# dusk-network/plonk_gadgets

Measured on AMD Instinct MI355X. Metric: gadget constraints/sec (range_check 256-bit), higher is better.
Workload: dtype u64x4 (BLS12-381 scalar, Montgomery limbs)

## Files before the change

### plonk_gadgets_amd/csrc/capi_composer.inc

```

struct RaggedBuffers {
    Scratch row_off, var_off, num_bits;
    uint64_t *rows() const { return row_off.as<uint64_t>(); }
    uint64_t *vars() const { return var_off.as<uint64_t>(); }
    uint32_t *bits() const { return num_bits.as<uint32_t>(); }
};

struct pg_composer {
    pg_engine *e = nullptr;
    hipStream_t stream = nullptr;
    uint64_t n = 0, nvars = 0, zero_var = 0;
    ColumnStore cols;
    Scratch d_stage;
    uint64_t *stage_words() const { return d_stage.as<uint64_t>(); }
    std::vector<uint64_t> pi_gate;
    std::vector<pg_scalar> pi_val;
    std::vector<pg::FourthWire> fourth;
    std::vector<pg::RangeSeg> range_segs;
    std::vector<pg::PermSeg> segs;
    Scratch perm_small, perm_big, val_ws;
    Scratch perm_pieces;
    std::vector<RaggedBuffers> ragged;
    Pinned h_total;
    uint64_t *totals() const { return h_total.as<uint64_t>(); }
// ... 1404 lines not shown
    if (np) {
        PG_TRY(B.take(d_gate, np * 8));
        PG_TRY(B.take(d_val, np * 32));
        PG_HIP_TRY(hipMemcpyAsync(*d_gate, c->pi_gate.data(), np * 8, hipMemcpyHostToDevice, c->stream));
        PG_HIP_TRY(hipMemcpyAsync(*d_val, c->pi_val.data(), np * 32, hipMemcpyHostToDevice, c->stream));
    }
    if (nf) {
        PG_TRY(B.take(d_fw, nf * sizeof(pg::FourthWire)));
        PG_HIP_TRY(hipMemcpyAsync(*d_fw, c->fourth.data(), nf * sizeof(pg::FourthWire), hipMemcpyHostToDevice, c->stream));
    }
    return PG_OK;
}

pg_status pg_composer_check(pg_composer *c, int64_t *first_bad) {
    if (!c || !first_bad) return fail(PG_ERR_INVALID_ARGUMENT, "NULL argument");
    PG_TRY(flush(c));
    PG_HIP_TRY(hipSetDevice(c->e->device));
    CallBuffers B(c->stream);
    uint64_t *d_gate; uint4 *d_val; pg::FourthWire *d_fw;
    PG_TRY(upload_sparse(c, B, &d_gate, &d_val, &d_fw));
    unsigned long long *d_bad = nullptr, h_bad = ~0ull;
    PG_TRY(B.take(&d_bad, 8));
    PG_HIP_TRY(hipMemcpyAsync(d_bad, &h_bad, 8, hipMemcpyHostToDevice, c->stream));
    const uint64_t want = (c->n + pg::kThreads - 1) / pg::kThreads;
    const uint32_t grid = (uint32_t)(want < (uint64_t)c->e->num_cus * 8 ? (want ? want : 1) : (uint64_t)c->e->num_cus * 8);
    hipLaunchKernelGGL(pg::check_kernel, dim3(grid), dim3(pg::kThreads), 0, c->stream, c->cols.view(), c->n, (uint64_t)0, c->nvars,
                       c->zero_var, d_gate, d_val, (uint32_t)c->pi_gate.size(), d_fw, (uint32_t)c->fourth.size(), d_bad);
    for (const pg::RangeSeg &s : c->range_segs) {
        const uint64_t rw = (s.items * s.g + pg::kThreads - 1) / pg::kThreads, most = (uint64_t)c->e->num_cus * 8;
        hipLaunchKernelGGL(pg::range_check_rows_kernel, dim3((uint32_t)(rw < most ? rw : most)), dim3(pg::kThreads), 0, c->stream, c->cols.view(), s,
                           c->nvars, d_bad);
    }
    PG_HIP_TRY(hipGetLastError());
    PG_HIP_TRY(hipMemcpyAsync(&h_bad, d_bad, 8, hipMemcpyDeviceToHost, c->stream));
    PG_HIP_TRY(hipStreamSynchronize(c->stream));
    *first_bad = h_bad == ~0ull ? -1 : (int64_t)h_bad;
    return PG_OK;
}

pg_status pg_composer_dense_pi(pg_composer *c, pg_scalar *d_out) {
    if (!c) return fail(PG_ERR_INVALID_ARGUMENT, "composer is NULL");
    PG_TRY(flush(c));
    PG_TRY(check_scalars(d_out, "d_out"));
    PG_HIP_TRY(hipSetDevice(c->e->device));
    PG_HIP_TRY(hipMemsetAsync(d_out, 0, c->n * 32, c->stream));
    CallBuffers B(c->stream);
    uint64_t *d_gate; uint4 *d_val; pg::FourthWire *d_fw;
    PG_TRY(upload_sparse(c, B, &d_gate, &d_val, &d_fw));
    const uint32_t np = (uint32_t)c->pi_gate.size();
    if (np) {
        hipLaunchKernelGGL(pg::scatter_pi_kernel, dim3((np + 255) / 256), dim3(256), 0, c->stream,
                           reinterpret_cast<uint4 *>(d_out), d_gate, d_val, np);
        PG_HIP_TRY(hipGetLastError());
    }
    PG_HIP_TRY(hipStreamSynchronize(c->stream));
    return PG_OK;
}

pg_status pg_composer_materialize(pg_composer *c, const pg_full_columns *out) {
    if (!c || !out) return fail(PG_ERR_INVALID_ARGUMENT, "NULL argument");
    PG_TRY(flush(c));
    PG_HIP_TRY(hipSetDevice(c->e->device));
    const uint32_t grid = (uint32_t)c->e->num_cus * 32;
    pg::MaterializeOut M{};
    pg_scalar *const consts[7] = {out->q_4, out->q_arith, out->q_range, out->q_logic, out->q_fixed_group_add,
                                  out->q_variable_group_add, out->w_4_value};
    for (int k = 0; k < 7; k++) {
        if (!consts[k]) continue;
        PG_TRY(check_scalars(consts[k], "constant column"));
        M.konst[k] = reinterpret_cast<uint4 *>(consts[k]);
    }
    pg_scalar *const vals[3] = {out->w_l_value, out->w_r_value, out->w_o_value};
    for (int i = 0; i < 3; i++) {
        if (!vals[i]) continue;
        PG_TRY(check_scalars(vals[i], "wire value column"));
        M.val[i] = reinterpret_cast<uint4 *>(vals[i]);
    }
    if (out->w_4) {
        PG_TRY(check_u64s(out->w_4, "w_4"));
        M.w_4 = out->w_4;
    }
    const auto generic = [&](uint64_t lo, uint64_t hi) {
        if (hi <= lo) return;
        const uint64_t want = (2 * (hi - lo) + 16383) / 16384;
        hipLaunchKernelGGL(pg::materialize_kernel, dim3((uint32_t)(want < grid ? want : grid)), dim3(pg::kThreads), 0, c->stream, c->cols.view(), M,
                           lo, hi, c->zero_var);
    };
    uint64_t at = 0;
#ifndef PG_MAT_GRID_PER_CU
#define PG_MAT_GRID_PER_CU 64
#endif
    using MatKernel = void (*)(const pg::ComposerCols, const pg::MaterializeOut, const pg::PermSeg, uint32_t, uint64_t);
    static const MatKernel self_ragged[2] = {pg::materialize_items_kernel<pg::MAT_SELF, pg::WIRES_MAX_BOUND, true>,
                                             pg::materialize_items_kernel<pg::MAT_SELF, pg::WIRES_MIX, true>};
    static const MatKernel read_wires = pg::materialize_items_kernel<pg::MAT_READ_WIRES, pg::WIRES_UNKNOWN>;
    static const MatKernel self[pg::WIRES_MIX + 1] = {
        nullptr,
        pg::materialize_items_kernel<pg::MAT_SELF, pg::WIRES_RANGE_CHECK>,
        pg::materialize_items_kernel<pg::MAT_SELF, pg::WIRES_MAX_BOUND>,
        pg::materialize_items_kernel<pg::MAT_SELF, pg::WIRES_RANGE_CHECK_ALLOCATED>,
        pg::materialize_items_kernel<pg::MAT_SELF, pg::WIRES_MAX_BOUND_ALLOCATED>,
        pg::materialize_items_kernel<pg::MAT_SELF, pg::WIRES_DECOMPOSITION>,
        pg::materialize_items_kernel<pg::MAT_SELF, pg::WIRES_MIX>,
    };
    for (const pg::PermSeg &s : c->segs) {
        const uint64_t group = pg::mat_group(s);
        const pg::MatRoute r = pg::mat_route(s, group);
        if (!r.windowed) continue;
        generic(at, s.gate_base);
        const uint64_t n_groups = (s.items + group - 1) / group, most = (uint64_t)c->e->num_cus * PG_MAT_GRID_PER_CU;
        const MatKernel kernel = r.mode != pg::MAT_SELF ? read_wires : r.ragged ? self_ragged[r.kind == pg::WIRES_MIX] : self[r.kind];
        hipLaunchKernelGGL(kernel, dim3((uint32_t)(n_groups < most ? n_groups : most)), dim3(pg::kMatThreads), 0, c->stream, c->cols.view(), M, s,
                           (uint32_t)group, c->zero_var);
        at = s.gate_end;
    }
    generic(at, c->n);
    CallBuffers B(c->stream);
    uint64_t *d_gate; uint4 *d_val; pg::FourthWire *d_fw;
    PG_TRY(upload_sparse(c, B, &d_gate, &d_val, &d_fw));
    if (d_fw)
        hipLaunchKernelGGL(pg::patch_fourth_kernel, dim3(1), dim3(64), 0, c->stream, reinterpret_cast<uint4 *>(out->q_4), out->w_4,
                           reinterpret_cast<uint4 *>(out->w_4_value), c->cols.view().vars, d_fw, (uint32_t)c->fourth.size());
    if (out->q_range)
        for (const pg::RangeSeg &s : c->range_segs) {
            const uint64_t rw = (2 * s.items * s.g + pg::kThreads - 1) / pg::kThreads;
            hipLaunchKernelGGL(pg::range_patch_kernel, dim3((uint32_t)(rw < grid ? rw : grid)), dim3(pg::kThreads), 0, c->stream,
                               reinterpret_cast<uint4 *>(out->q_range), s);
        }
    PG_HIP_TRY(hipGetLastError());
    PG_HIP_TRY(hipStreamSynchronize(c->stream));
    return PG_OK;
}

static pg_status perm_reserve(pg_composer *c, Scratch &buf, size_t bytes) {
    if (bytes <= buf.size()) return PG_OK;
    PG_HIP_TRY(hipStreamSynchronize(c->stream));
    return buf.reserve(bytes);
}

pg_status pg_composer_permutation_reserve(pg_composer *c, uint64_t sparse_positions) {
    if (!c) return fail(PG_ERR_INVALID_ARGUMENT, "composer is NULL");
    c->sparse_cap_first = sparse_positions;
    if (sparse_positions) c->perm_last_sparse = 0;
    return PG_OK;
}

static pg_status perm_kernel_attributes(pg_engine *e) {
    if (e->perm_attributes_set) return PG_OK;
    const void *const ladder_lds[4] = {
        reinterpret_cast<const void *>(pg::perm_ladder_kernel<false>), reinterpret_cast<const void *>(pg::perm_template_kernel<true>),
        reinterpret_cast<const void *>(pg::perm_template_kernel<false>), reinterpret_cast<const void *>(pg::perm_ladder_kernel<true>)};
    if (pg::kPermLadderLds)
        for (const void *k : ladder_lds) PG_HIP_TRY(hipFuncSetAttribute(k, hipFuncAttributeMaxDynamicSharedMemorySize, (int)pg::kPermLadderLds));
    PG_HIP_TRY(hipFuncSetAttribute(reinterpret_cast<const void *>(pg::perm_identity_kernel), hipFuncAttributeMaxDynamicSharedMemorySize,
                                   (int)pg::kPermIdentityLds));
    e->perm_attributes_set = true;
    return PG_OK;
}

pg_status pg_composer_permutation(pg_composer *c, uint64_t padded_n, uint64_t *d_sigma) {
    if (!c) return fail(PG_ERR_INVALID_ARGUMENT, "composer is NULL");
    PG_TRY(flush(c));
    PG_TRY(check_u64s(d_sigma, "d_sigma"));
    if (padded_n < c->n) return fail(PG_ERR_INVALID_ARGUMENT, "padded_n is smaller than the circuit");
    PG_HIP_TRY(hipSetDevice(c->e->device));
    PG_TRY(perm_kernel_attributes(c->e));
    const uint32_t grid = (uint32_t)c->e->num_cus * 32;
    uint32_t pos_bits = 2, var_bits = 1;
    while ((1ull << pos_bits) < 4 * c->n) pos_bits++;
    while ((1ull << var_bits) < c->nvars + 1) var_bits++;
    if (pos_bits + var_bits > 64) return fail(PG_ERR_INVALID_ARGUMENT, "circuit too large for 64-bit (Variable, position) keys");
    std::vector<pg::PermSeg> segs;
    std::vector<pg::PermRoute> routes;
    std::vector<std::pair<uint64_t, uint64_t>> gaps;
    uint64_t at = 0, gap_rows = 0;
    for (pg::PermSeg s : c->segs) {
        const pg::PermRoute route = pg::perm_route(s);
        if (!(s.group = pg::perm_group(s, route))) continue;
        if (s.gate_base > at) gaps.emplace_back(at, s.gate_base);
        segs.push_back(s);
        routes.push_back(route);
        at = s.gate_end;
    }
    if (c->n > at) gaps.emplace_back(at, c->n);
    for (const auto &g : gaps) gap_rows += g.second - g.first;
    const size_t seg_bytes = round256(segs.size() * sizeof(pg::PermSeg));
    const size_t fw_bytes = round256(c->fourth.size() * sizeof(pg::FourthWire));
    PG_TRY(perm_reserve(c, c->perm_small, seg_bytes + fw_bytes + 256));
    char *small = c->perm_small.as<char>();
    pg::PermCtx X;
    X.C = c->cols.view(); X.n = c->n; X.padded_n = padded_n; X.zero_var = c->zero_var;
    X.segs = reinterpret_cast<const pg::PermSeg *>(small); X.n_segs = (uint32_t)segs.size();
    X.fw = reinterpret_cast<const pg::FourthWire *>(small + seg_bytes); X.n_fw = (uint32_t)c->fourth.size();
    X.fw_lo = 0; X.fw_span = 0; X.pos_bits = pos_bits;
    X.hole_key = pos_bits + var_bits >= 64 ? ~0ull : (1ull << (pos_bits + var_bits)) - 1;
    if (!c->fourth.empty()) {
        uint64_t lo = ~0ull, hi = 0;
        for (const pg::FourthWire &f : c->fourth) { lo = f.gate < lo ? f.gate : lo; hi = f.gate > hi ? f.gate : hi; }
        X.fw_lo = lo; X.fw_span = hi - lo;
    }
    uint64_t reserved = 0, total_pieces = 0;
    for (size_t i = 0; i < segs.size(); i++) {
        if (pg::perm_reserves_slots(routes[i])) {
            segs[i].sparse_base = reserved;
            reserved += segs[i].items * pg::perm_slots_per_item(segs[i], routes[i]);
        }
        if (pg::perm_needs_piece_items(routes[i])) total_pieces += pg::perm_pieces(segs[i]);
    }
    if (total_pieces) {
        PG_TRY(perm_reserve(c, c->perm_pieces, total_pieces * sizeof(uint32_t)));
        uint32_t *at_piece = c->perm_pieces.as<uint32_t>();
        for (size_t i = 0; i < segs.size(); i++) {
            if (!pg::perm_needs_piece_items(routes[i])) continue;
            pg::PermSeg &s = segs[i];
            s.piece_item = at_piece;
            at_piece += pg::perm_pieces(s);
            const uint64_t want = (s.items + pg::kThreads - 1) / pg::kThreads;
            hipLaunchKernelGGL(pg::perm_piece_items_kernel, dim3((uint32_t)(want < grid ? want : grid)), dim3(pg::kThreads), 0, c->stream, s,
                               pg::kPermLadderRows, at_piece - pg::perm_pieces(s));
        }
        PG_HIP_TRY(hipGetLastError());
    }
    unsigned long long *d_count = reinterpret_cast<unsigned long long *>(small + seg_bytes + fw_bytes);
    if (!segs.empty())
        PG_HIP_TRY(hipMemcpyAsync(small, segs.data(), segs.size() * sizeof(pg::PermSeg), hipMemcpyHostToDevice, c->stream));
    if (!c->fourth.empty())
        PG_HIP_TRY(hipMemcpyAsync(small + seg_bytes, c->fourth.data(), c->fourth.size() * sizeof(pg::FourthWire),
                                  hipMemcpyHostToDevice, c->stream));
    uint64_t cap = c->sparse_cap_first ? c->sparse_cap_first : 4 * gap_rows + c->sparse_hint + (1ull << 16), nS = 0;
    if (cap < c->perm_last_sparse) cap = c->perm_last_sparse;
    uint64_t *k0 = nullptr, *k1 = nullptr, holes = 0;
    size_t tmp_bytes = 0;
    for (int attempt = 0;; attempt++) {
        uint64_t *nul = nullptr;
        PG_HIP_TRY(rocprim::radix_sort_keys(nullptr, tmp_bytes, nul, nul, (size_t)cap, 0u, pos_bits + var_bits, c->stream));
        const size_t kb = round256(cap * 8);
        PG_TRY(perm_reserve(c, c->perm_big, 2 * kb + tmp_bytes + 256));
        k0 = c->perm_big.as<uint64_t>();
        k1 = reinterpret_cast<uint64_t *>(c->perm_big.as<char>() + kb);
        const pg::PermSparse Q{k0, d_count, cap};
        hipLaunchKernelGGL(pg::perm_count_init_kernel, dim3(1), dim3(1), 0, c->stream, d_count, reserved);
        for (size_t i = 0; i < segs.size(); i++) {
            const pg::PermSeg &s = segs[i];
            const uint64_t most = (uint64_t)c->e->num_cus * 64, pieces = pg::perm_pieces(s);
            const uint32_t lds = pg::perm_lds_bytes(s, routes[i]);
            if (routes[i] != pg::PERM_ITEMS && routes[i] != pg::PERM_LADDER && pieces > 0x7fffffffull)
                return fail(PG_ERR_INVALID_ARGUMENT, "segment too large for one launch");
            switch (routes[i]) {
            case pg::PERM_LADDER: {
                const uint64_t lmost = pg::kPermLadderRows <= 2048 ? 0x7fffffffull : most;
                hipLaunchKernelGGL(pg::perm_ladder_kernel<false>, dim3((uint32_t)(pieces < lmost ? pieces : lmost)), dim3(pg::kThreads), lds,
                                   c->stream, X, s, Q, d_sigma);
                break;
            }
            case pg::PERM_LADDER_RAGGED:
                hipLaunchKernelGGL(pg::perm_ladder_kernel<true>, dim3((uint32_t)pieces), dim3(pg::kThreads), lds, c->stream, X, s, Q, d_sigma);
                break;
            case pg::PERM_TEMPLATE:
                hipLaunchKernelGGL(pg::perm_template_kernel<false>, dim3((uint32_t)pieces), dim3(pg::kThreads), lds, c->stream, X, s,
                                   pg::template_rows(s.wire_kind), Q, d_sigma);
                break;
            case pg::PERM_TEMPLATE_RAGGED:
                hipLaunchKernelGGL(pg::perm_template_kernel<true>, dim3((uint32_t)pieces), dim3(pg::kThreads), lds, c->stream, X, s,
                                   pg::template_rows(s.wire_kind), Q, d_sigma);
                break;
            case pg::PERM_ITEMS: {
                const uint64_t groups = (s.items + s.group - 1) / s.group;
                hipLaunchKernelGGL(pg::perm_item_kernel, dim3((uint32_t)(groups < most ? groups : most)), dim3(pg::kThreads), lds, c->stream, X, s,
                                   groups, Q, d_sigma);
                break;
            }
            }
        }
        for (const auto &g : gaps) {
            const uint64_t nblk = (g.second - g.first + pg::kPermChunk - 1) / pg::kPermChunk;
            hipLaunchKernelGGL(pg::perm_gap_kernel, dim3((uint32_t)nblk), dim3(pg::kThreads), 0, c->stream, X, g.first, g.second, Q,
                               d_sigma);
        }
        PG_HIP_TRY(hipMemcpyAsync(c->totals(), d_count, 16, hipMemcpyDeviceToHost, c->stream));
        PG_HIP_TRY(hipStreamSynchronize(c->stream));
        nS = c->totals()[0];
        holes = c->totals()[1];
        c->perm_last_sparse = nS;
        if (nS <= cap) break;
        if (attempt) return fail(PG_ERR_HIP, "sparse position list grew between two passes");
        cap = nS;
    }
    if (nS) {
        PG_HIP_TRY(rocprim::radix_sort_keys(c->perm_big.as<char>() + 2 * round256(cap * 8), tmp_bytes, k0, k1,
                                            (size_t)nS, 0u, pos_bits + var_bits, c->stream));
        nS -= holes;
    }
    if (nS) {
        const uint64_t want = (nS + pg::kThreads - 1) / pg::kThreads;
        hipLaunchKernelGGL(pg::perm_sparse_link_kernel, dim3((uint32_t)(want < grid ? want : grid)), dim3(pg::kThreads), 0, c->stream,
                           X, k1, nS, d_sigma);
        if (!segs.empty()) {
            const uint64_t wantw = (nS + 255) / 256;
            hipLaunchKernelGGL(pg::perm_splice_kernel, dim3((uint32_t)(wantw < grid ? wantw : grid)), dim3(pg::kThreads), 0, c->stream,
                               X, k1, nS, d_sigma);
        }
    }
    if (padded_n > c->n) {
        const uint64_t per_run = ((padded_n - c->n) / 2 + 1 + pg::kPermIdentityUnits - 1) / pg::kPermIdentityUnits;
        if (4 * per_run > 0x7fffffffull) return fail(PG_ERR_INVALID_ARGUMENT, "padding too large for one launch");
        hipLaunchKernelGGL(pg::perm_identity_kernel, dim3((uint32_t)(4 * per_run)), dim3(pg::kThreads), pg::kPermIdentityLds, c->stream,
                           d_sigma, c->n, padded_n);
    }
    PG_HIP_TRY(hipGetLastError());
    return PG_OK;
}

pg_status pg_check_rows(pg_engine *e, const pg_columns *cols, uint64_t n_gates, uint64_t var_base, uint64_t n_vars,
                        pg_variable zero_var, int64_t *first_bad, void *stream) {
    if (!e || !first_bad) return fail(PG_ERR_INVALID_ARGUMENT, "NULL argument");
    *first_bad = -1;
    if (n_gates == 0) return PG_OK;
    PG_TRY(check_columns(cols));
    PG_HIP_TRY(hipSetDevice(e->device));
    hipStream_t st = static_cast<hipStream_t>(stream);
    pg::ComposerCols C;
    C.q[0] = reinterpret_cast<uint4 *>(cols->q_m); C.q[1] = reinterpret_cast<uint4 *>(cols->q_l);
    C.q[2] = reinterpret_cast<uint4 *>(cols->q_r); C.q[3] = reinterpret_cast<uint4 *>(cols->q_o);
    C.q[4] = reinterpret_cast<uint4 *>(cols->q_c);
    C.w[0] = cols->w_l; C.w[1] = cols->w_r; C.w[2] = cols->w_o;
    C.vars = reinterpret_cast<uint4 *>(cols->var_values);
    unsigned long long *d_bad = nullptr, h_bad = ~0ull;
    CallBuffers B(st);
    PG_TRY(B.take(&d_bad, 8));
    PG_HIP_TRY(hipMemcpyAsync(d_bad, &h_bad, 8, hipMemcpyHostToDevice, st));
    hipLaunchKernelGGL(pg::check_kernel, dim3((uint32_t)e->num_cus * 16), dim3(pg::kThreads), 0, st, C, n_gates, var_base, n_vars,
                       zero_var, (const uint64_t *)nullptr, (const uint4 *)nullptr, 0u, (const pg::FourthWire *)nullptr, 0u, d_bad);
    hipError_t le = hipGetLastError();
    if (le == hipSuccess) le = hipMemcpyAsync(&h_bad, d_bad, 8, hipMemcpyDeviceToHost, st);
    if (le == hipSuccess) le = hipStreamSynchronize(st);
    if (le != hipSuccess) return fail(PG_ERR_HIP, std::string("pg_check_rows: ") + hipGetErrorString(le));
    *first_bad = h_bad == ~0ull ? -1 : (int64_t)h_bad;
    return PG_OK;
}

}
```

### plonk_gadgets_amd/csrc/experiment.hpp

```cpp
#pragma once

#if !defined(PG_EXPERIMENT) &&                                                                                                  \
    (defined(PG_NT_STORES) || defined(PG_FULL_BARRIERS) || defined(PG_EMIT_WAVES_PER_SIMD) || defined(PG_XCD_REMAP) ||          \
     defined(PG_UNALIGNED_SWEEPS) || defined(PG_ROWS_WAVES_PER_SIMD) || defined(PG_ROWS_SETPRIO) || defined(PG_INVERT_FERMAT) || \
     defined(PG_INV_GRP) || defined(PG_RC_W) || defined(PG_MB_W) || defined(PG_MIX_VARS_VGPRS) || defined(PG_MIX_STAMPS) ||     \
     defined(PG_QUEUE_MAX) || defined(PG_PERM_LDS_PAD) || defined(PG_GRID_BLOCKS_PER_CU) || defined(PG_PLAN_TWO_LAUNCHES) ||    \
     defined(PG_INV_LANES_PER_CU) || defined(PG_INV_MAX_PER_LANE) || defined(PG_SIDE_STREAM_NORMAL_PRIORITY) || defined(PG_VAR_SWEEP_SINGLE) || \
     defined(PG_TILE_SPREAD) || defined(PG_MIX_EARLY_TILES) || defined(PG_MAT_THREADS) || defined(PG_MAT_UNROLL) || defined(PG_MAT_LOADS) || defined(PG_PERM_LADDER_ROWS) || defined(PG_PERM_LADDER_LDS) || defined(PG_MAT_GRID_PER_CU) || defined(PG_EMIT_GRID_BLOCKS_PER_CU) || \
     defined(PG_MSM_SMALL_WINDOW))
#error "a PG_... build option is defined without -DPG_EXPERIMENT: the shipped library is built with none of them (csrc/experiment.hpp)"
#endif
```

### plonk_gadgets_amd/csrc/footprint.hpp

```cpp
#pragma once

#include <cstdint>

#if defined(__HIPCC__)
#define PG_FOOTPRINT_HD __host__ __device__
#else
#define PG_FOOTPRINT_HD
#endif

namespace pg {

struct PermSeg {
    uint64_t gate_base, gate_end, var_base, var_end;
    uint32_t L, V;
    uint64_t items;
    const uint64_t *row_off, *var_off;
    uint32_t group;
    uint32_t wire_kind, wire_n;
    uint64_t sparse_base;
    uint32_t tail;
    const uint32_t *piece_item;
};
enum : uint32_t { WIRES_UNKNOWN = 0, WIRES_RANGE_CHECK = 1, WIRES_MAX_BOUND = 2, WIRES_RANGE_CHECK_ALLOCATED = 3, WIRES_MAX_BOUND_ALLOCATED = 4,
                  WIRES_DECOMPOSITION = 5,
                  WIRES_MIX = 6,
                  WIRES_SELECT_ZERO = 7, WIRES_SELECT_ONE = 8, WIRES_MAYBE_EQUAL = 9, WIRES_IS_NON_ZERO = 10, WIRES_GATE_OUT = 11,
                  WIRES_GATE_ROWS = 12, WIRES_KINDS = 13 };

PG_FOOTPRINT_HD inline uint32_t ladder_foreign_per_item(uint32_t kind) {
    return kind == WIRES_RANGE_CHECK_ALLOCATED ? 4u : kind == WIRES_MAX_BOUND_ALLOCATED ? 2u : kind == WIRES_DECOMPOSITION ? 1u : 0u;
}
PG_FOOTPRINT_HD inline uint32_t template_foreign_per_item(uint32_t kind) {
    return kind == WIRES_SELECT_ZERO || kind == WIRES_MAYBE_EQUAL || kind == WIRES_IS_NON_ZERO || kind == WIRES_GATE_OUT ? 2u
           : kind == WIRES_SELECT_ONE || kind == WIRES_GATE_ROWS ? 3u : 0u;
}
PG_FOOTPRINT_HD inline bool is_template_kind(uint32_t kind) { return kind >= WIRES_MIX && kind < WIRES_KINDS; }

struct KindShape {
    uint16_t rows, rows_per_bit, vars, vars_per_bit;
    uint8_t allocated_twin;
};
constexpr KindShape kKindShapes[WIRES_KINDS] = {
    {0, 0, 0, 0, 0},
    {11, 4, 524, 2, WIRES_RANGE_CHECK_ALLOCATED},
    {5, 2, 262, 1, WIRES_MAX_BOUND_ALLOCATED},
    {11, 4, 523, 2, 0},
    {5, 2, 261, 1, 0},
    {4, 2, 260, 1, 0},
    {10, 0, 15, 0, 0},
    {1, 0, 1, 0, 0},
    {4, 0, 4, 0, 0},
    {3, 0, 3, 0, 0},
    {3, 0, 3, 0, 0},
    {1, 0, 1, 0, 0},
    {1, 0, 0, 0, 0},
};
constexpr uint32_t kind_rows(uint32_t kind, uint64_t n = 0) { return kKindShapes[kind].rows + kKindShapes[kind].rows_per_bit * (uint32_t)n; }
constexpr uint32_t kind_vars(uint32_t kind, uint64_t n = 0) { return kKindShapes[kind].vars + kKindShapes[kind].vars_per_bit * (uint32_t)n; }
constexpr uint32_t ladder_kind(uint32_t fused_kind, bool fused) { return fused ? fused_kind : kKindShapes[fused_kind].allocated_twin; }
inline uint32_t kind_foreign(uint32_t kind) { return is_template_kind(kind) ? template_foreign_per_item(kind) : ladder_foreign_per_item(kind); }
inline uint32_t kind_sparse_hint(uint32_t kind) { return kind == WIRES_DECOMPOSITION ? 2u : kind_foreign(kind); }

inline PermSeg footprint(uint64_t gate0, uint64_t var0, uint64_t items, uint32_t wire_kind, uint32_t wire_n = 0, uint32_t tail = 0) {
    const uint32_t L = kind_rows(wire_kind, wire_n) + tail, V = kind_vars(wire_kind, wire_n);
    return PermSeg{gate0, gate0 + items * L, var0, var0 + items * V, L, V, items, nullptr, nullptr, 1, wire_kind, wire_n, 0, tail, nullptr};
}

constexpr uint32_t kFootprintMinRows = 4096;

constexpr uint32_t kPermLocalLdsLimit = 64 * 1024 - 256;
constexpr uint32_t kPermNone = 0xFFFF, kPermDone = 0xFFFE;
PG_FOOTPRINT_HD inline uint32_t perm_local_lds_bytes(uint32_t L, uint32_t V) {
    return 4 * V + 2 * (V + 2) + 2 * (3 * L + 3 * L + L) + L + 16;
}
#ifndef PG_PERM_LADDER_ROWS
#define PG_PERM_LADDER_ROWS 512
#endif
#ifndef PG_PERM_LADDER_LDS
#define PG_PERM_LADDER_LDS 39936
#endif
#ifndef PG_PERM_LDS_PAD
#define PG_PERM_LDS_PAD 0
#endif
constexpr uint32_t kPermLadderRows = PG_PERM_LADDER_ROWS;
constexpr uint32_t kPermLadderLds = PG_PERM_LADDER_LDS;

enum PermRoute : uint32_t {
    PERM_ITEMS = 0,
    PERM_LADDER,
    PERM_LADDER_RAGGED,
    PERM_TEMPLATE,
    PERM_TEMPLATE_RAGGED,
};
inline PermRoute perm_route(const PermSeg &s) {
    if (s.wire_kind != WIRES_UNKNOWN && !s.row_off && s.wire_n >= 2) return PERM_LADDER;
    if (is_template_kind(s.wire_kind) && s.tail == 0) return s.row_off ? PERM_TEMPLATE_RAGGED : PERM_TEMPLATE;
    if (s.row_off && s.wire_kind == WIRES_MAX_BOUND && s.tail == 0) return PERM_LADDER_RAGGED;
    return PERM_ITEMS;
}
inline bool perm_fits(const PermSeg &s, uint64_t k) {
    return 4 * k * s.L < kPermDone && k * s.V < kPermNone && perm_local_lds_bytes((uint32_t)(k * s.L), (uint32_t)(k * s.V)) <= kPermLocalLdsLimit;
}
inline uint32_t perm_group(const PermSeg &s, PermRoute route) {
    if (!perm_fits(s, 1)) return 0;
    if (route == PERM_LADDER ? !is_template_kind(s.wire_kind) || s.tail == 0 : route != PERM_ITEMS) return 1;
    uint64_t k = 1024 / s.L;
    k = k < 1 ? 1 : (k > s.items ? s.items : k);
    while (k > 1 && !perm_fits(s, k)) k--;
    return (uint32_t)k;
}
inline bool perm_reserves_slots(PermRoute route) { return route == PERM_LADDER || route == PERM_TEMPLATE || route == PERM_TEMPLATE_RAGGED; }
inline uint32_t perm_slots_per_item(const PermSeg &s, PermRoute route) {
    return route == PERM_LADDER ? ladder_foreign_per_item(s.wire_kind) : perm_reserves_slots(route) ? template_foreign_per_item(s.wire_kind) : 0u;
}
inline bool perm_needs_piece_items(PermRoute route) { return route == PERM_LADDER_RAGGED || route == PERM_TEMPLATE_RAGGED; }
inline uint64_t perm_pieces(const PermSeg &s) { return (s.gate_end - (s.gate_base & ~1ull) + kPermLadderRows - 1) / kPermLadderRows; }
inline uint32_t perm_lds_bytes(const PermSeg &s, PermRoute route) {
    switch (route) {
    case PERM_LADDER: return ladder_foreign_per_item(s.wire_kind) ? 0u : kPermLadderLds;
    case PERM_LADDER_RAGGED: return kPermLadderLds;
    case PERM_TEMPLATE:
    case PERM_TEMPLATE_RAGGED: return template_foreign_per_item(s.wire_kind) ? 0u : kPermLadderLds - 8192;
    default: return perm_local_lds_bytes(s.group * s.L, s.group * s.V) + PG_PERM_LDS_PAD;
    }
}

constexpr uint32_t kMatWindowVars = 1040;
enum : int {
    MAT_READ_WIRES = 0,
    MAT_SELF = 2,
};
constexpr uint32_t kMatWitItems = 4;
constexpr uint32_t kMatMixRaggedItems = 127;

inline uint64_t mat_group(const PermSeg &s) {
    const uint64_t group = kMatWindowVars / (s.V ? s.V : 1);
    return group < 1 ? 1 : (group > s.items ? s.items : group);
}
struct MatRoute {
    bool windowed;
    int mode;
    uint32_t kind;
    bool ragged;
};
inline MatRoute mat_route(const PermSeg &s, uint64_t group) {
    if (s.V > kMatWindowVars || s.V == 0 || s.gate_end - s.gate_base < kFootprintMinRows) return MatRoute{false, MAT_READ_WIRES, WIRES_UNKNOWN, false};
    if (s.row_off) {
        if (s.wire_kind == WIRES_MAX_BOUND && group <= kMatWitItems) return MatRoute{true, MAT_SELF, WIRES_MAX_BOUND, true};
        if (s.wire_kind == WIRES_MIX && group < kMatMixRaggedItems) return MatRoute{true, MAT_SELF, WIRES_MIX, true};
        return MatRoute{true, MAT_READ_WIRES, WIRES_UNKNOWN, false};
    }
    if (s.wire_kind != WIRES_UNKNOWN && s.wire_kind <= WIRES_MIX && (ladder_foreign_per_item(s.wire_kind) == 0 || group <= kMatWitItems))
        return MatRoute{true, MAT_SELF, s.wire_kind, false};
    return MatRoute{true, MAT_READ_WIRES, WIRES_UNKNOWN, false};
}

}
```

### plonk_gadgets_amd/csrc/permutation.hpp

```cpp
#pragma once

#include <cstring>

#include <rocprim/rocprim.hpp>

#include "composer.hpp"
#include "footprint.hpp"
#include "range_gadgets.hpp"

namespace pg {

constexpr uint32_t kZeroWire = 0xfffffffeu;
__device__ __forceinline__ void seg_wire_offsets(uint32_t kind, uint32_t n, uint32_t j, uint32_t off[3], uint32_t tail = 0) {
    const uint32_t x0 = kind == WIRES_RANGE_CHECK || kind == WIRES_MAX_BOUND ? 1u : 0u;
    if (tail && kind >= WIRES_RANGE_CHECK && kind <= WIRES_MAX_BOUND_ALLOCATED) {
        const bool rc = kind == WIRES_RANGE_CHECK || kind == WIRES_RANGE_CHECK_ALLOCATED;
        const uint32_t own = rc ? 4 * n + 11 : 2 * n + 5, res = x0 + (rc ? 2 * n + 522 : n + 260);
        if (j >= own) {
            off[0] = off[1] = off[2] = res;
            return;
        }
    }
    if (kind == WIRES_MIX) {
        constexpr uint64_t lo = 0xF50ull | 0x777ull << 12 | 0x760ull << 24 | 0x888ull << 36 | 0x921ull << 48;
// ... 332 lines not shown
    }
    const uint32_t open = ladder_block_row(j, n, j2, w2);
    if (j == 0) {
        if (kind == WIRES_MAX_BOUND_ALLOCATED) return 3;
        j2[0] = 0; w2[0] = 1; j2[1] = 0; w2[1] = 0;
    } else if (open == 2) { j2[1] = 0; w2[1] = 2; }
    else if (open == 1) { j2[0] = tail ? L : 2 * n + 3; w2[0] = tail ? 0 : 2; }
    return 0;
}

__device__ __forceinline__ uint32_t ladder_foreign_wires(uint32_t kind, uint32_t n, uint32_t j) {
    if (kind == WIRES_RANGE_CHECK_ALLOCATED) return j == 0 || j == 2 * n + 5 ? 3u : 0u;
    if (kind == WIRES_MAX_BOUND_ALLOCATED) return j == 0 ? 3u : 0u;
    if (kind == WIRES_DECOMPOSITION) return j == 2 * n + 1 ? 2u : 0u;
    return 0u;
}

__device__ __forceinline__ uint32_t ladder_foreign_rank(uint32_t kind, uint32_t j, uint32_t w) {
    if (kind == WIRES_DECOMPOSITION) return 0u;
    return (j ? 2u : 0u) + w;
}

constexpr uint32_t kPermRaggedWindow = 64;
__global__ __launch_bounds__(kThreads) void perm_piece_items_kernel(const PermSeg S, uint32_t rows_per_piece, uint32_t *piece_item) {
    const uint64_t d = S.gate_base & 1;
    for (uint64_t i = (uint64_t)blockIdx.x * kThreads + threadIdx.x; i < S.items; i += (uint64_t)gridDim.x * kThreads) {
        const uint64_t r0 = S.row_off[i], r1 = S.row_off[i + 1];
        if (i == 0) piece_item[0] = 0;
        for (uint64_t p = (r0 + d + rows_per_piece - 1) / rows_per_piece; p * rows_per_piece < r1 + d; p++)
            if (p) piece_item[p] = (uint32_t)i;
    }
}

template <bool RAGGED>
__global__ __launch_bounds__(kThreads) void perm_ladder_kernel(const PermCtx X, const PermSeg S, const PermSparse Q, uint64_t *sigma) {
    extern __shared__ uint4 perm_ladder_pad[];
    __shared__ uint32_t s_off[RAGGED ? kPermRaggedWindow : 1];
    static_assert(!RAGGED || kPermLadderRows / 9 + 3 <= kPermRaggedWindow, "a piece's items fit the window of prefix sums");
    const uint32_t lane = threadIdx.x & 63, kind = S.wire_kind;
    uint32_t n = S.wire_n;
    if (X.padded_n == 1) perm_ladder_pad[threadIdx.x] = make_uint4(0, 0, 0, 0);
    const uint64_t first = S.gate_base & ~1ull, total = S.gate_end - first;
    const bool wide = (reinterpret_cast<uintptr_t>(sigma) & 15) == 0 && !(X.padded_n & 1);
    const uint32_t recip = (uint32_t)(((1ull << 32) + S.L - 1) / S.L);
    const bool pow2 = (X.padded_n & (X.padded_n - 1)) == 0;
    const uint32_t sh = 63u - (uint32_t)__clzll((long long)X.padded_n);
    auto enc = [&](uint64_t gate, uint32_t wire) { return pow2 ? ((uint64_t)wire << sh) + gate : perm_encode(gate, wire, X.padded_n); };
    auto zero_wires = [&](uint64_t g, uint32_t j) {
        uint32_t z = 0;
        for (uint32_t m = ladder_foreign_wires(kind, n, j); m; m &= m - 1) {
            const uint32_t w = (uint32_t)__ffs((int)m) - 1;
            if (X.C.w[w][g] == X.zero_var) z |= 1u << w;
        }
        return z;
    };
    for (uint64_t base = (uint64_t)blockIdx.x * kPermLadderRows; base < total; base += (uint64_t)gridDim.x * kPermLadderRows) {
        const uint64_t g_first = first + base, rel = g_first < S.gate_base ? 0 : g_first - S.gate_base;
        uint64_t item0, rows0 = 0;
        if constexpr (RAGGED) {
            item0 = S.piece_item[base / kPermLadderRows];
            rows0 = S.row_off[item0];
            __syncthreads();
            if (threadIdx.x < kPermRaggedWindow) {
                const uint64_t i = item0 + threadIdx.x < S.items ? item0 + threadIdx.x : S.items;
                s_off[threadIdx.x] = (uint32_t)(S.row_off[i] - rows0);
            }
            __syncthreads();
        } else {
            item0 = rel / S.L;
            rows0 = item0 * S.L;
        }
        const uint32_t j0 = (uint32_t)(rel - rows0), skip = (uint32_t)(g_first < S.gate_base ? S.gate_base - g_first : 0);
        for (uint32_t t = 2 * threadIdx.x; t < kPermLadderRows; t += 2 * kThreads) {
            uint64_t out[4][2], fitem[2] = {0, 0};
            uint32_t foreign[2] = {0, 0}, fslots[2] = {0, 0}, fj[2] = {0, 0};
            bool live[2];
#pragma unroll
            for (uint32_t h = 0; h < 2; h++) {
                const uint64_t g = g_first + t + h;
                live[h] = g >= S.gate_base && g < S.gate_end;
                const uint32_t tt = t + h - skip;
                uint32_t q, j;
                uint64_t g_item;
#pragma unroll
                for (uint32_t w = 0; w < 4; w++) out[w][h] = 0;
                if constexpr (RAGGED) {
                    if (!live[h]) continue;
                    const uint32_t x = j0 + tt;
                    uint32_t lo = 0;
#pragma unroll
                    for (uint32_t step = kPermRaggedWindow / 2; step; step >>= 1)
                        if (s_off[lo + step] <= x) lo += step;
                    q = lo;
                    j = x - s_off[lo];
                    n = (s_off[lo + 1] - s_off[lo] - 5) >> 1;
                    g_item = S.gate_base + rows0 + s_off[lo];
                } else {
                    q = __umulhi(j0 + tt, recip);
                    j = (j0 + tt) - q * S.L;
                    g_item = S.gate_base + (item0 + q) * S.L;
                }
                if (!live[h]) continue;
                uint32_t j2[3], w2[3];
                const uint32_t fw = ladder_row(kind, n, j, j2, w2, S.tail), zw = fw ? zero_wires(g, j) : 0u;
                foreign[h] = fw & ~zw;
                fslots[h] = fw;
                fitem[h] = item0 + q;
                fj[h] = j;
#pragma unroll
                for (uint32_t w = 0; w < 3; w++) {
                    if (fw >> w & 1) {
                        const uint32_t later = (zw | 8u) & ~((2u << w) - 1);
                        out[w][h] = enc(g, (uint32_t)__ffs((int)later) - 1);
                    } else {
                        out[w][h] = enc(g_item + j2[w], w2[w]);
                    }
                }
                if (g + 1 < S.gate_end) {
                    const uint32_t jn = j + 1 == S.L ? 0 : j + 1;
                    const uint32_t zn = ladder_foreign_wires(kind, n, jn) ? zero_wires(g + 1, jn) : 0u;
                    out[3][h] = enc(g + 1, (uint32_t)__ffs((int)(zn | 8u)) - 1);
                } else {
                    out[3][h] = perm_next_zero_from(X, S.gate_end);
                }
            }
            const uint64_t g = g_first + t;
#pragma unroll
            for (uint32_t w = 0; w < 4; w++) {
                const bool skip0 = !live[0] || (foreign[0] >> w & 1), skip1 = !live[1] || (foreign[1] >> w & 1);
                uint64_t *dst = sigma + enc(g, w);
                if (wide && !skip0 && !skip1)
                    store16(reinterpret_cast<uint4 *>(dst), make_uint4((uint32_t)out[w][0], (uint32_t)(out[w][0] >> 32), (uint32_t)out[w][1],
                                                                      (uint32_t)(out[w][1] >> 32)));
                else {
                    if (!skip0) dst[0] = out[w][0];
                    if (!skip1) dst[1] = out[w][1];
                }
            }
            if (fslots[0] | fslots[1]) {
                const uint32_t F = ladder_foreign_per_item(kind);
#pragma unroll
                for (uint32_t h = 0; h < 2; h++)
                    for (uint32_t m = fslots[h]; m; m &= m - 1) {
                        const uint32_t w = (uint32_t)__ffs((int)m) - 1;
                        const uint64_t at = S.sparse_base + fitem[h] * F + ladder_foreign_rank(kind, fj[h], w);
                        if (foreign[h] >> w & 1) perm_sparse_put(X, Q, at, X.C.w[w][g + h], g + h, w);
                        else {
                            if (at < Q.cap) Q.keys[at] = X.hole_key;
                            atomicAdd(Q.count + 1, 1ull);
                        }
                    }
            }
        }
    }
}

constexpr uint8_t kTmplForeign = 0xF0, kTmplZero = 0xFE, kTmplNone = 0xFF;
constexpr uint32_t kTmplRows = 10;
struct SegTemplate {
    uint8_t L[2], V[2];
    uint8_t wire[2][kTmplRows][3];
};
#define PG_T3(a, b, c) {a, b, c}
#define PG_TF0 0xF0
#define PG_TF1 0xF1
#define PG_TF2 0xF2
#define PG_TZ 0xFE
#define PG_TX PG_T3(0xFF, 0xFF, 0xFF)
constexpr SegTemplate kSegTemplates[WIRES_KINDS - WIRES_MIX] = {
    {{10, 8}, {15, 13},
     {{PG_T3(0, 5, PG_TZ), PG_T3(7, 7, 7), PG_T3(0, 6, 7), PG_T3(8, 8, 8), PG_T3(1, 2, 9), PG_T3(8, 2, 10), PG_T3(9, 10, 11), PG_T3(3, 4, 12),
       PG_T3(13, 12, 14), PG_T3(14, 12, 12)},
      {PG_T3(0, 5, PG_TZ), PG_T3(6, 6, 6), PG_T3(1, 2, 7), PG_T3(6, 2, 8), PG_T3(7, 8, 9), PG_T3(3, 4, 10), PG_T3(11, 10, 12), PG_T3(12, 10, 10),
       PG_TX, PG_TX}}},
    {{1, 0}, {1, 0}, {{PG_T3(PG_TF0, PG_TF1, 0), PG_TX, PG_TX, PG_TX, PG_TX, PG_TX, PG_TX, PG_TX, PG_TX, PG_TX}, {PG_TX, PG_TX, PG_TX, PG_TX, PG_TX, PG_TX, PG_TX, PG_TX, PG_TX, PG_TX}}},
    {{4, 0}, {4, 0}, {{PG_T3(0, 0, 0), PG_T3(PG_TF0, PG_TF1, 1), PG_T3(0, PG_TF1, 2), PG_T3(1, 2, 3), PG_TX, PG_TX, PG_TX, PG_TX, PG_TX, PG_TX}, {PG_TX, PG_TX, PG_TX, PG_TX, PG_TX, PG_TX, PG_TX, PG_TX, PG_TX, PG_TX}}},
    {{3, 0}, {3, 0}, {{PG_T3(PG_TF0, PG_TF1, 0), PG_T3(1, 0, 2), PG_T3(2, 0, 0), PG_TX, PG_TX, PG_TX, PG_TX, PG_TX, PG_TX, PG_TX}, {PG_TX, PG_TX, PG_TX, PG_TX, PG_TX, PG_TX, PG_TX, PG_TX, PG_TX, PG_TX}}},
    {{3, 1}, {3, 1}, {{PG_T3(PG_TF0, 0, PG_TZ), PG_T3(2, 2, 2), PG_T3(PG_TF0, 1, 2), PG_TX, PG_TX, PG_TX, PG_TX, PG_TX, PG_TX, PG_TX}, {PG_T3(PG_TF0, 0, PG_TZ), PG_TX, PG_TX, PG_TX, PG_TX, PG_TX, PG_TX, PG_TX, PG_TX, PG_TX}}},
    {{1, 0}, {1, 0}, {{PG_T3(PG_TF0, PG_TF1, 0), PG_TX, PG_TX, PG_TX, PG_TX, PG_TX, PG_TX, PG_TX, PG_TX, PG_TX}, {PG_TX, PG_TX, PG_TX, PG_TX, PG_TX, PG_TX, PG_TX, PG_TX, PG_TX, PG_TX}}},
    {{1, 0}, {0, 0}, {{PG_T3(PG_TF0, PG_TF1, PG_TF2), PG_TX, PG_TX, PG_TX, PG_TX, PG_TX, PG_TX, PG_TX, PG_TX, PG_TX}, {PG_TX, PG_TX, PG_TX, PG_TX, PG_TX, PG_TX, PG_TX, PG_TX, PG_TX, PG_TX}}},
};
#undef PG_T3
#undef PG_TF0
#undef PG_TF1
#undef PG_TF2
#undef PG_TZ
#undef PG_TX
constexpr bool seg_templates_match_kind_shapes(uint32_t k = WIRES_MIX) {
    return k == WIRES_KINDS || (kSegTemplates[k - WIRES_MIX].L[0] == kind_rows(k) && kSegTemplates[k - WIRES_MIX].V[0] == kind_vars(k) &&
                                seg_templates_match_kind_shapes(k + 1));
}
static_assert(seg_templates_match_kind_shapes(), "footprint.hpp's kKindShapes and kSegTemplates agree about a full item");

struct TemplateRows {
    uint64_t row[2][kTmplRows];
    uint8_t L[2], V[2], F[2];
    uint8_t Fmax, pad;
};
inline TemplateRows template_rows(uint32_t kind) {
    const SegTemplate &T = kSegTemplates[kind - WIRES_MIX];
    TemplateRows R{};
    for (uint32_t sh = 0; sh < 2; sh++) {
        R.L[sh] = T.L[sh];
        R.V[sh] = T.V[sh];
        uint32_t foreign = 0;
        const uint32_t n = (uint32_t)T.L[sh] * 3;
        for (uint32_t p = 0; p < n; p++) {
            const uint8_t code = T.wire[sh][p / 3][p % 3];
            uint64_t b = 0;
            if (code < kTmplForeign) {
                uint32_t first = 0xff, next = 0xff;
                for (uint32_t q = 0; q < n; q++)
                    if (T.wire[sh][q / 3][q % 3] == code) {
                        if (first == 0xff) first = q;
                        if (q > p && next == 0xff) next = q;
                    }
                const uint32_t z = next != 0xff ? next : first;
                b = 1u | (uint64_t)code << 2 | (uint64_t)(4 * (z / 3) + z % 3) << 6;
            } else if (code < kTmplZero) {
                b = 2u | (uint64_t)foreign++ << 12;
            } else if (code == kTmplZero) {
                b = 3u;
            }
            R.row[sh][p / 3] |= b << (16 * (p % 3));
        }
        R.F[sh] = (uint8_t)foreign;
    }
    R.Fmax = (uint8_t)template_foreign_per_item(kind);
    return R;
}

constexpr uint32_t kTmplWindow = 1024;
template <bool RAGGED>
__global__ __launch_bounds__(kThreads) void perm_template_kernel(const PermCtx X, const PermSeg S, const TemplateRows T, const PermSparse Q,
                                                                uint64_t *sigma) {
    extern __shared__ uint4 perm_template_pad[];
    __shared__ uint64_t s_row[2][kTmplRows];
    __shared__ uint32_t s_off[RAGGED ? kTmplWindow : 1];
    static_assert(kPermLadderRows + 3 <= kTmplWindow, "a piece's items fit the window of prefix sums");
    if (X.padded_n == 1) perm_template_pad[threadIdx.x] = make_uint4(0, 0, 0, 0);
    const uint32_t Lf = T.L[0], Ls = T.L[1], Fmax = T.Fmax, Ff = T.F[0], Fs = T.F[1];
    if (threadIdx.x < 2 * kTmplRows) s_row[threadIdx.x / kTmplRows][threadIdx.x % kTmplRows] = T.row[threadIdx.x / kTmplRows][threadIdx.x % kTmplRows];
    __syncthreads();
    const uint64_t first = S.gate_base & ~1ull, total = S.gate_end - first;
    const bool wide = (reinterpret_cast<uintptr_t>(sigma) & 15) == 0 && !(X.padded_n & 1);
    const uint32_t recip = (uint32_t)(((1ull << 32) + Lf - 1) / Lf);
    const bool pow2 = (X.padded_n & (X.padded_n - 1)) == 0;
    const uint32_t sh_bits = 63u - (uint32_t)__clzll((long long)X.padded_n);
    auto enc = [&](uint64_t gate, uint32_t wire) { return pow2 ? ((uint64_t)wire << sh_bits) + gate : perm_encode(gate, wire, X.padded_n); };
    for (uint64_t base = (uint64_t)blockIdx.x * kPermLadderRows; base < total; base += (uint64_t)gridDim.x * kPermLadderRows) {
        const uint64_t g_first = first + base, rel = g_first < S.gate_base ? 0 : g_first - S.gate_base;
        uint64_t item0, rows0;
        if constexpr (RAGGED) {
            item0 = S.piece_item[base / kPermLadderRows];
            rows0 = S.row_off[item0];
            __syncthreads();
            for (uint32_t e = threadIdx.x; e < kTmplWindow; e += kThreads) {
                const uint64_t i = item0 + e < S.items ? item0 + e : S.items;
                s_off[e] = (uint32_t)(S.row_off[i] - rows0);
            }
            __syncthreads();
        } else {
            item0 = rel / Lf;
            rows0 = item0 * Lf;
        }
        const uint32_t j0 = (uint32_t)(rel - rows0), skip = (uint32_t)(g_first < S.gate_base ? S.gate_base - g_first : 0);
        struct Row { uint32_t item, j, sh, rows; uint64_t g_item, word; };
        auto locate = [&](uint32_t x, Row &R) {
            if constexpr (RAGGED) {
                uint32_t lo = 0;
#pragma unroll
                for (uint32_t step = kTmplWindow / 2; step; step >>= 1)
                    if (s_off[lo + step] <= x) lo += step;
                R.item = lo;
                R.j = x - s_off[lo];
                R.rows = s_off[lo + 1] - s_off[lo];
                R.sh = R.rows == Lf ? 0u : 1u;
                R.g_item = S.gate_base + rows0 + s_off[lo];
            } else {
                R.item = Lf == 1 ? x : __umulhi(x, recip);
                R.j = x - R.item * Lf;
                R.sh = 0;
                R.rows = Lf;
                R.g_item = S.gate_base + rows0 + (uint64_t)R.item * Lf;
            }
            R.word = s_row[R.sh][R.j];
        };
        auto step = [&](Row &R) {
            if (R.j + 1 < R.rows) R.j++;
            else {
                R.g_item += R.rows;
                R.item++;
                R.j = 0;
                if constexpr (RAGGED) {
                    R.rows = s_off[R.item + 1] - s_off[R.item];
                    R.sh = R.rows == Lf ? 0u : 1u;
                }
            }
            R.word = s_row[R.sh][R.j];
        };
        auto zero_mask = [&](uint64_t g, uint64_t word) {
            uint32_t z = 0;
#pragma unroll
            for (uint32_t w = 0; w < 3; w++) {
                const uint32_t type = (uint32_t)(word >> (16 * w)) & 3u;
                if (type == 3u) z |= 1u << w;
// ... 171 lines not shown
```

Baseline: 32.78 billion.

## Add column-wise ladder permutation kernel using affine per-class successor tables

Adds a new kernel path for range-check and max-bound ladder segments. Each block handles one of the four wire columns over a run of gates and computes sigma successors from a small per-class table whose offsets are affine in the ladder length. That table is built and validated on the device, and a failure flag is returned to the host. The aim is to replace the per-piece ladder_row evaluation and its LDS staging with cheap table lookups, and to write coalesced 16-byte sigma stores per column. In exchange it adds a class-table launch, a larger readback and a runtime correctness check that fails the call if the affine assumption breaks.

```diff
diff --git a/plonk_gadgets_amd/csrc/capi_composer.inc b/plonk_gadgets_amd/csrc/capi_composer.inc
--- a/plonk_gadgets_amd/csrc/capi_composer.inc
+++ b/plonk_gadgets_amd/csrc/capi_composer.inc
@@ -1580,6 +1580,10 @@
         reinterpret_cast<const void *>(pg::perm_template_kernel<false>), reinterpret_cast<const void *>(pg::perm_ladder_kernel<true>)};
     if (pg::kPermLadderLds)
         for (const void *k : ladder_lds) PG_HIP_TRY(hipFuncSetAttribute(k, hipFuncAttributeMaxDynamicSharedMemorySize, (int)pg::kPermLadderLds));
+    const void *const column_lds[2] = {reinterpret_cast<const void *>(pg::perm_ladder_column_kernel<false>),
+                                       reinterpret_cast<const void *>(pg::perm_ladder_column_kernel<true>)};
+    if (pg::kPermColumnLds)
+        for (const void *k : column_lds) PG_HIP_TRY(hipFuncSetAttribute(k, hipFuncAttributeMaxDynamicSharedMemorySize, (int)pg::kPermColumnLds));
     PG_HIP_TRY(hipFuncSetAttribute(reinterpret_cast<const void *>(pg::perm_identity_kernel), hipFuncAttributeMaxDynamicSharedMemorySize,
                                    (int)pg::kPermIdentityLds));
     e->perm_attributes_set = true;
@@ -1614,7 +1618,8 @@
     for (const auto &g : gaps) gap_rows += g.second - g.first;
     const size_t seg_bytes = round256(segs.size() * sizeof(pg::PermSeg));
     const size_t fw_bytes = round256(c->fourth.size() * sizeof(pg::FourthWire));
-    PG_TRY(perm_reserve(c, c->perm_small, seg_bytes + fw_bytes + 256));
+    const size_t class_bytes = round256(2 * pg::kPermClassStride * sizeof(int32_t));
+    PG_TRY(perm_reserve(c, c->perm_small, seg_bytes + fw_bytes + 256 + class_bytes));
     char *small = c->perm_small.as<char>();
     pg::PermCtx X;
     X.C = c->cols.view(); X.n = c->n; X.padded_n = padded_n; X.zero_var = c->zero_var;
@@ -1650,6 +1655,10 @@
         PG_HIP_TRY(hipGetLastError());
     }
     unsigned long long *d_count = reinterpret_cast<unsigned long long *>(small + seg_bytes + fw_bytes);
+    const pg::PermClassTables classes{reinterpret_cast<int32_t *>(small + seg_bytes + fw_bytes + 256), d_count + 2};
+    bool any_columns = false;
+    for (size_t i = 0; i < segs.size(); i++) any_columns = any_columns || pg::perm_ladder_columns(segs[i], routes[i]);
+    if (any_columns) hipLaunchKernelGGL(pg::perm_class_table_kernel, dim3(1), dim3(64), 0, c->stream, classes);
     if (!segs.empty())
         PG_HIP_TRY(hipMemcpyAsync(small, segs.data(), segs.size() * sizeof(pg::PermSeg), hipMemcpyHostToDevice, c->stream));
     if (!c->fourth.empty())
@@ -1674,14 +1683,26 @@
             const uint32_t lds = pg::perm_lds_bytes(s, routes[i]);
             if (routes[i] != pg::PERM_ITEMS && routes[i] != pg::PERM_LADDER && pieces > 0x7fffffffull)
                 return fail(PG_ERR_INVALID_ARGUMENT, "segment too large for one launch");
+            const bool columns = pg::perm_ladder_columns(s, routes[i]);
+            const uint32_t column_blocks = (uint32_t)(4 * ((s.gate_end - (s.gate_base & ~1ull) + pg::kPermColumnRun - 1) / pg::kPermColumnRun));
             switch (routes[i]) {
             case pg::PERM_LADDER: {
+                if (columns) {
+                    hipLaunchKernelGGL(pg::perm_ladder_column_kernel<false>, dim3(column_blocks), dim3(pg::kThreads), pg::kPermColumnLds, c->stream,
+                                       X, s, classes.word, d_sigma);
+                    break;
+                }
                 const uint64_t lmost = pg::kPermLadderRows <= 2048 ? 0x7fffffffull : most;
                 hipLaunchKernelGGL(pg::perm_ladder_kernel<false>, dim3((uint32_t)(pieces < lmost ? pieces : lmost)), dim3(pg::kThreads), lds,
                                    c->stream, X, s, Q, d_sigma);
                 break;
             }
             case pg::PERM_LADDER_RAGGED:
+                if (columns) {
+                    hipLaunchKernelGGL(pg::perm_ladder_column_kernel<true>, dim3(column_blocks), dim3(pg::kThreads), pg::kPermColumnLds, c->stream,
+                                       X, s, classes.word, d_sigma);
+                    break;
+                }
                 hipLaunchKernelGGL(pg::perm_ladder_kernel<true>, dim3((uint32_t)pieces), dim3(pg::kThreads), lds, c->stream, X, s, Q, d_sigma);
                 break;
             case pg::PERM_TEMPLATE:
@@ -1705,8 +1726,9 @@
             hipLaunchKernelGGL(pg::perm_gap_kernel, dim3((uint32_t)nblk), dim3(pg::kThreads), 0, c->stream, X, g.first, g.second, Q,
                                d_sigma);
         }
-        PG_HIP_TRY(hipMemcpyAsync(c->totals(), d_count, 16, hipMemcpyDeviceToHost, c->stream));
+        PG_HIP_TRY(hipMemcpyAsync(c->totals(), d_count, 24, hipMemcpyDeviceToHost, c->stream));
         PG_HIP_TRY(hipStreamSynchronize(c->stream));
+        if (any_columns && c->totals()[2]) return fail(PG_ERR_HIP, "ladder_row is not affine in the ladder length on some class of rows");
         nS = c->totals()[0];
         holes = c->totals()[1];
         c->perm_last_sparse = nS;
diff --git a/plonk_gadgets_amd/csrc/experiment.hpp b/plonk_gadgets_amd/csrc/experiment.hpp
--- a/plonk_gadgets_amd/csrc/experiment.hpp
+++ b/plonk_gadgets_amd/csrc/experiment.hpp
@@ -7,6 +7,6 @@
      defined(PG_QUEUE_MAX) || defined(PG_PERM_LDS_PAD) || defined(PG_GRID_BLOCKS_PER_CU) || defined(PG_PLAN_TWO_LAUNCHES) ||    \
      defined(PG_INV_LANES_PER_CU) || defined(PG_INV_MAX_PER_LANE) || defined(PG_SIDE_STREAM_NORMAL_PRIORITY) || defined(PG_VAR_SWEEP_SINGLE) || \
      defined(PG_TILE_SPREAD) || defined(PG_MIX_EARLY_TILES) || defined(PG_MAT_THREADS) || defined(PG_MAT_UNROLL) || defined(PG_MAT_LOADS) || defined(PG_PERM_LADDER_ROWS) || defined(PG_PERM_LADDER_LDS) || defined(PG_MAT_GRID_PER_CU) || defined(PG_EMIT_GRID_BLOCKS_PER_CU) || \
-     defined(PG_MSM_SMALL_WINDOW))
+     defined(PG_MSM_SMALL_WINDOW) || defined(PG_PERM_COLUMN_RUN) || defined(PG_PERM_COLUMN_LDS) || defined(PG_PERM_COLUMNS))
 #error "a PG_... build option is defined without -DPG_EXPERIMENT: the shipped library is built with none of them (csrc/experiment.hpp)"
 #endif
diff --git a/plonk_gadgets_amd/csrc/footprint.hpp b/plonk_gadgets_amd/csrc/footprint.hpp
--- a/plonk_gadgets_amd/csrc/footprint.hpp
+++ b/plonk_gadgets_amd/csrc/footprint.hpp
@@ -84,6 +84,19 @@
 #endif
 constexpr uint32_t kPermLadderRows = PG_PERM_LADDER_ROWS;
 constexpr uint32_t kPermLadderLds = PG_PERM_LADDER_LDS;
+#ifndef PG_PERM_COLUMN_RUN
+#define PG_PERM_COLUMN_RUN 2048
+#endif
+#ifndef PG_PERM_COLUMN_LDS
+#define PG_PERM_COLUMN_LDS 19456
+#endif
+#ifndef PG_PERM_COLUMNS
+#define PG_PERM_COLUMNS 1
+#endif
+constexpr uint32_t kPermColumnRun = PG_PERM_COLUMN_RUN;
+constexpr uint32_t kPermColumnLds = PG_PERM_COLUMN_LDS;
+constexpr bool kPermColumns = PG_PERM_COLUMNS;
+static_assert(kPermColumnRun % kPermLadderRows == 0 && kPermColumnRun % 512 == 0, "a column run is whole pieces and whole passes of 256 lanes x 2 gates");
 
 enum PermRoute : uint32_t {
     PERM_ITEMS = 0,
diff --git a/plonk_gadgets_amd/csrc/permutation.hpp b/plonk_gadgets_amd/csrc/permutation.hpp
--- a/plonk_gadgets_amd/csrc/permutation.hpp
+++ b/plonk_gadgets_amd/csrc/permutation.hpp
@@ -508,6 +508,173 @@
                     }
             }
         }
+    }
+}
+
+constexpr uint32_t kPermBlockClasses = 11;
+constexpr uint32_t kPermClassesRc = 2 * kPermBlockClasses + 1, kPermClassesMb = kPermBlockClasses;
+constexpr uint32_t kPermClassStride = 72;
+struct PermClassTables {
+    int32_t *word;
+    unsigned long long *bad;
+};
+__device__ __forceinline__ uint32_t ladder_block_class(uint32_t jj, uint32_t n) {
+    const uint32_t d = 2 * n + 4 - jj;
+    return jj < 4 ? jj : d <= 4 ? 4 + d : 9 + (jj & 1);
+}
+__device__ __forceinline__ uint32_t ladder_class(bool rc, uint32_t n, uint32_t j) {
+    if (!rc) return ladder_block_class(j, n);
+    const uint32_t L = 2 * n + 5, blk = j >= L ? 1u : 0u;
+    return j == 2 * L ? 2 * kPermBlockClasses : blk * kPermBlockClasses + ladder_block_class(j - blk * L, n);
+}
+__device__ __forceinline__ uint32_t ladder_class_row(bool rc, uint32_t n, uint32_t c) {
+    const uint32_t L = 2 * n + 5;
+    if (rc && c == 2 * kPermBlockClasses) return 2 * L;
+    const uint32_t blk = c >= kPermBlockClasses ? 1u : 0u, cc = c - blk * kPermBlockClasses;
+    return blk * L + (cc < 4 ? cc : cc < 9 ? 2 * n + 8 - cc : cc - 5);
+}
+__global__ __launch_bounds__(64) void perm_class_table_kernel(const PermClassTables T) {
+    if (threadIdx.x == 0) *T.bad = 0;
+    __syncthreads();
+    const bool rc = threadIdx.x < kPermClassesRc;
+    const uint32_t c = rc ? threadIdx.x : threadIdx.x - kPermClassesRc;
+    if (!rc && c >= kPermClassesMb) return;
+    const uint32_t kind = rc ? WIRES_RANGE_CHECK : WIRES_MAX_BOUND, ns[3] = {8, 9, 11};
+    int32_t d[3][3];
+    uint32_t w[3][3];
+    bool ok = true;
+    for (uint32_t k = 0; k < 3; k++) {
+        const uint32_t j = ladder_class_row(rc, ns[k], c);
+        uint32_t j2[3];
+        ok = ok && ladder_class(rc, ns[k], j) == c && ladder_row(kind, ns[k], j, j2, w[k]) == 0;
+        for (uint32_t x = 0; x < 3; x++) d[k][x] = (int32_t)j2[x] - (int32_t)j;
+    }
+    for (uint32_t x = 0; x < 3; x++) {
+        const int32_t b = d[1][x] - d[0][x], a = d[0][x] - 8 * b;
+        ok = ok && d[2][x] == a + 11 * b && w[0][x] == w[1][x] && w[0][x] == w[2][x] && w[0][x] < 3 && b >= -32 && b < 32;
+        T.word[(rc ? 0 : kPermClassStride) + 3 * c + x] = (int32_t)((uint32_t)a << 8 | (uint32_t)(b + 32) << 2 | w[0][x]);
+    }
+    if (!ok) *T.bad = 1;
+}
+
+inline bool perm_ladder_columns(const PermSeg &s, PermRoute route) {
+    if (!kPermColumns || (s.gate_end - (s.gate_base & ~1ull) + kPermColumnRun - 1) / kPermColumnRun > 0x1fffffffull) return false;
+    if (route == PERM_LADDER_RAGGED) return true;
+    return route == PERM_LADDER && (s.wire_kind == WIRES_RANGE_CHECK || s.wire_kind == WIRES_MAX_BOUND) && s.tail == 0;
+}
+constexpr uint32_t perm_pow2_at_least(uint32_t x, uint32_t p = 1) { return p >= x ? p : perm_pow2_at_least(x, 2 * p); }
+constexpr uint32_t kPermColumnWindow = perm_pow2_at_least(kPermColumnRun / 9 + 3);
+
+template <bool RAGGED>
+__global__ __launch_bounds__(kThreads) void perm_ladder_column_kernel(const PermCtx X, const PermSeg S, const int32_t *table, uint64_t *sigma) {
+    extern __shared__ uint4 perm_column_pad[];
+    __shared__ int32_t s_tab[kPermClassesRc];
+    __shared__ uint32_t s_off[RAGGED ? kPermColumnWindow : 1];
+    if (X.padded_n == 1) perm_column_pad[threadIdx.x] = make_uint4(0, 0, 0, 0);
+    const uint32_t col = blockIdx.x & 3;
+    const bool rc = !RAGGED && S.wire_kind == WIRES_RANGE_CHECK;
+    const uint64_t first = S.gate_base & ~1ull;
+    const uint64_t g_first = first + (uint64_t)(blockIdx.x >> 2) * kPermColumnRun;
+    const bool wide = (reinterpret_cast<uintptr_t>(sigma) & 15) == 0 && !(X.padded_n & 1);
+    const bool pow2 = (X.padded_n & (X.padded_n - 1)) == 0;
+    const uint32_t sh = 63u - (uint32_t)__clzll((long long)X.padded_n);
+    auto enc = [&](uint64_t gate, uint32_t wire) { return pow2 ? ((uint64_t)wire << sh) + gate : perm_encode(gate, wire, X.padded_n); };
+    auto put = [&](uint64_t g, bool live0, bool live1, uint64_t out0, uint64_t out1) {
+        uint64_t *dst = sigma + enc(g, col);
+        if (wide && live0 && live1)
+            store16(reinterpret_cast<uint4 *>(dst), make_uint4((uint32_t)out0, (uint32_t)(out0 >> 32), (uint32_t)out1, (uint32_t)(out1 >> 32)));
+        else {
+            if (live0) dst[0] = out0;
+            if (live1) dst[1] = out1;
+        }
+    };
+    if (col == 3) {
+#pragma unroll
+        for (uint32_t k = 0; k < kPermColumnRun / (2 * kThreads); k++) {
+            const uint64_t g = g_first + 2 * (k * kThreads + threadIdx.x);
+            uint64_t out[2];
+#pragma unroll
+            for (uint32_t h = 0; h < 2; h++) {
+                out[h] = enc(g + h + 1, 3);
+                if (g + h + 1 == S.gate_end) out[h] = perm_next_zero_from(X, S.gate_end);
+            }
+            put(g, g >= S.gate_base && g < S.gate_end, g + 1 < S.gate_end, out[0], out[1]);
+        }
+        return;
+    }
+    const uint32_t classes = rc ? kPermClassesRc : kPermClassesMb;
+    if (threadIdx.x < classes) {
+        const int32_t e = table[(rc ? 0 : kPermClassStride) + 3 * threadIdx.x + col];
+        const int32_t delta = (e >> 8) + ((int32_t)(e >> 2 & 63) - 32) * (int32_t)S.wire_n;
+        s_tab[threadIdx.x] = RAGGED ? e : (int32_t)((uint32_t)delta << 2 | (uint32_t)(e & 3));
+    }
+    const uint64_t rel = g_first < S.gate_base ? 0 : g_first - S.gate_base;
+    uint64_t rows0;
+    if constexpr (RAGGED) {
+        const uint64_t item0 = S.piece_item[(uint64_t)(blockIdx.x >> 2) * (kPermColumnRun / kPermLadderRows)];
+        rows0 = S.row_off[item0];
+        for (uint32_t e = threadIdx.x; e < kPermColumnWindow; e += kThreads) {
+            const uint64_t i = item0 + e < S.items ? item0 + e : S.items;
+            s_off[e] = (uint32_t)(S.row_off[i] - rows0);
+        }
+    } else {
+        rows0 = rel >> 32 ? rel / S.L * S.L : (uint64_t)((uint32_t)rel / S.L) * S.L;
+    }
+    __syncthreads();
+    const uint32_t j0 = (uint32_t)(rel - rows0), skip = (uint32_t)(g_first < S.gate_base ? S.gate_base - g_first : 0);
+    const uint32_t recip = (uint32_t)(((1ull << 32) + S.L - 1) / S.L);
+    static_assert(kPermColumnRun <= 8192, "x = j0 + t < L + kPermColumnRun with L < 2^11: x L < 2^32");
+    struct Row { uint32_t j, rows, n, at; };
+    auto locate = [&](uint32_t x, Row &R) {
+        if constexpr (RAGGED) {
+            uint32_t lo = 0;
+#pragma unroll
+            for (uint32_t step = kPermColumnWindow / 2; step; step >>= 1)
+                if (s_off[lo + step] <= x) lo += step;
+            R.at = lo;
+            R.j = x - s_off[lo];
+            R.rows = s_off[lo + 1] - s_off[lo];
+            R.n = (R.rows - 5) >> 1;
+        } else {
+            R.at = 0;
+            R.j = x - __umulhi(x, recip) * S.L;
+            R.rows = S.L;
+            R.n = S.wire_n;
+        }
+    };
+    auto step = [&](Row &R) {
+        if (++R.j < R.rows) return;
+        R.j = 0;
+        if constexpr (RAGGED) {
+            R.at++;
+            R.rows = s_off[R.at + 1] - s_off[R.at];
+            R.n = (R.rows - 5) >> 1;
+        }
+    };
+    auto successor = [&](uint64_t g, const Row &R) {
+        const int32_t e = s_tab[ladder_class(rc, R.n, R.j)];
+        const int32_t delta = RAGGED ? (e >> 8) + ((int32_t)(e >> 2 & 63) - 32) * (int32_t)R.n : e >> 2;
+        return enc(g + (uint64_t)(int64_t)delta, (uint32_t)(e & 3));
+    };
+#pragma unroll
+    for (uint32_t k = 0; k < kPermColumnRun / (2 * kThreads); k++) {
+        const uint32_t t = 2 * (k * kThreads + threadIdx.x);
+        const uint64_t g = g_first + t;
+        const bool live0 = g >= S.gate_base && g < S.gate_end, live1 = g + 1 < S.gate_end;
+        uint64_t out0 = 0, out1 = 0;
+        Row R;
+        if (live0) {
+            locate(j0 + t - skip, R);
+            out0 = successor(g, R);
+            if (live1) {
+                step(R);
+                out1 = successor(g + 1, R);
+            }
+        } else if (live1) {
+            locate(j0 + t + 1 - skip, R);
+            out1 = successor(g + 1, R);
+        }
+        put(g, live0, live1, out0, out1);
     }
 }
 
```

Result: no change. 32.73 billion (-0.1%).
